# 192459/lmc-atomi

Hardware: AMD Instinct MI355X
Metric: lmc_chain_iterations_per_s (higher is better)
Workload: dtype f32; 1 GPU; 512x512 MYULA deblur (5x5 uniform box blur, sigma=0.75) + isotropic TV prox K=10 (tau_reg=0.3), 1024 chains/GPU x 1 GPU, Philox noise, x0=0, posterior moments every 1 it; chains_per_gpu=1024, chains_total=1024, tv_iters=10, sampler=MYULA (algs.py:477-587), parallelism=chains sharded x1, collective=none

## Files before the change

### lmc_atomi_amd/csrc/lmc_host.h

```cpp
#pragma once
#include <string>
#include <vector>

#include "lmc_launch.h"

namespace lmc::host {

int fail(int code, const char* fmt, ...);

#define HIP_TRY(expr)                                                                          \
  do {                                                                                         \
    hipError_t e_ = (expr);                                                                    \
    if (e_ != hipSuccess) return fail(LMC_E_HIP, "%s failed: %s", #expr, hipGetErrorString(e_)); \
  } while (0)

inline hipStream_t S(void* s) { return reinterpret_cast<hipStream_t>(s); }

inline bool eprox_params_ok(int kind, float p0, float p1) {
  static const unsigned char nonneg[] = {1, 1, 1, 1, 1, 1, 1, 3, 1, 1, 3, 1, 1, 0, 0};
  return (!(nonneg[kind] & 1) || p0 >= 0.f) && (!(nonneg[kind] & 2) || p1 >= 0.f);
}

struct Problem {
  int H = 0, W = 0;
  int data_kind = 0;
  int wl2 = 0;
  int pois = 0;
  float sigma_f = 0.f;
  const float* y = nullptr;
  const float* mask = nullptr;
  lmc::BlurTaps taps{};
  int prior_kind = 0;
  float prior_sigma = 0.f;
  int tv_niter = 0;
  float tv_step = 0.125f;
  float betas[lmc::kMaxTvIters] = {};
  int ncvx_kind = 0;
  float ncvx_lambda = 0.f, ncvx_gamma = 1.f;
  int ncvx_niter = 0;
  int ncvx_aniso = 0;
  int tv_warm = 0;
  int tv_warm_asked = 0;
  int tv_niter_asked = 0;
  float tv_rtol = 0.f;
  float ncvx_rtol = 0.f;
  int tv_exit_path = 0;
  int iters_per_launch = 0, moments_overlap = 0, moments_bg_wgs = 0;
  int cheb_pair = 1;
  int eprox_kind = 0, eprox_mask = 0;
  float eprox_p0 = 0.f, eprox_p1 = 0.f;
  const float* prox_scale = nullptr;
  int64_t prox_scale_cs = 0, prox_scale_ps = 0;
  int box = 0;
  float box_lo = 0.f, box_hi = 0.f;
  int variant = 0;
  float implicit_tol = 0.f;
};

struct RtState {
  int* kc = nullptr;
  int* start = nullptr;
  int* pred = nullptr;
  double* obj = nullptr;
  unsigned long long* reruns = nullptr;
  int stride = 0;
  size_t n = 0;
  hipError_t need(size_t n_img, int niter) {
    if (n_img <= n && niter + 1 <= stride) return hipSuccess;
    release();
    hipError_t e = hipMalloc(&kc, sizeof(int) * n_img);
    if (e == hipSuccess) e = hipMalloc(&start, sizeof(int) * n_img);
    if (e == hipSuccess) e = hipMalloc(&pred, sizeof(int) * n_img);
    if (e == hipSuccess) e = hipMalloc(&obj, sizeof(double) * n_img * (size_t)(niter + 1));
    if (e == hipSuccess) e = hipMalloc(&reruns, sizeof(unsigned long long) * 4);
    if (e == hipSuccess) e = hipMemset(pred, 0, sizeof(int) * n_img);
    if (e == hipSuccess) e = hipMemset(reruns, 0, sizeof(unsigned long long) * 4);
    if (e == hipSuccess) { n = n_img; stride = niter + 1; }
    return e;
  }
  void release() {
    if (kc) (void)hipFree(kc);
    if (start) (void)hipFree(start);
    if (pred) (void)hipFree(pred);
    if (obj) (void)hipFree(obj);
    if (reruns) (void)hipFree(reruns);
    kc = start = pred = nullptr; obj = nullptr; reruns = nullptr; n = 0; stride = 0;
  }
};

// ... 164 lines not shown
```

### lmc_atomi_amd/csrc/lmc_step_pipe.hip

```cpp
#include "lmc_step_pipe_kernel.h"

namespace lmc {

int centred_blur_taps(const StepArgs& a, float* uc, float* vc);

bool pipe_geometry_ok(const StepArgs& a) {
  if (a.prior_kind != LMC_PRIOR_TV_ISO || a.prox_ext) return false;
  if (a.W <= 128 || a.H < 1 || a.W > 16384) return false;
  if (a.W > 512 && (a.f_out || a.g_out)) return false;
  if ((a.W & (a.W > 256 ? 7 : 3)) && !(a.tv.niter == 10 || (a.tv.niter >= 20 && a.tv.niter % 10 == 0))) return false;
  if (a.data_kind == LMC_DATA_BLUR) {
    float uc[kMaxBlur], vc[kMaxBlur];
    if (centred_blur_taps(a, uc, vc) == 0) return false;
  } else if (a.data_kind != LMC_DATA_NONE && a.data_kind != LMC_DATA_IDENTITY && a.data_kind != LMC_DATA_MASK) {
    return false;
  }
  if (a.data_kind != LMC_DATA_BLUR && (a.ncvx_kind != LMC_NCVX_NONE || a.f_out)) return false;
  return true;
}

int pipe_links(const StepArgs& a) {
  if (a.prior_kind != LMC_PRIOR_TV_ISO || a.tv.niter > kMaxTvIters) return 0;
  const int n = a.tv.niter;
  const bool single = n == 2 || n == 6 || n == 8 || n == 9 || n == 10;
  if (!single && (n < 19 || (n % 10 != 0 && n % 10 != 9))) return 0;
  if (a.tv_aniso && (n % 10 != 0 || a.f_out || a.g_out)) return 0;
  if (a.box && (n % 10 != 0 || a.f_out || a.g_out || a.tv_aniso)) return 0;
  if (a.pois && (n != 10 || a.f_out || a.g_out || a.tv_aniso || a.ncvx_kind != LMC_NCVX_NONE || a.extra)) return 0;
  if (a.wl2 && (n != 10 || a.f_out || a.g_out || a.tv_aniso || a.ncvx_kind != LMC_NCVX_NONE || a.extra || a.data_kind == LMC_DATA_MASK)) return 0;
  if (a.tv_in || a.tv_out || a.tv_state_only || a.tv_warm) return 0;
  if (!pipe_geometry_ok(a)) return 0;
  return single ? 1 : (n + 9) / 10;
}

bool pipe_supported(const StepArgs& a) { return pipe_links(a) == 1; }

bool pipe_warm_supported(const StepArgs& a) {
  const int n = a.tv.niter;
  if (!(n == 1 || n == 2 || n == 3) || a.tv_aniso || a.box || a.pois || a.wl2) return false;
  return pipe_geometry_ok(a);
}

int pipe_taps(StepArgs& a) {
  int KT = 0;
  if (a.data_kind == LMC_DATA_BLUR) {
    float uc[kMaxBlur] = {0}, vc[kMaxBlur] = {0};
    KT = centred_blur_taps(a, uc, vc);
    for (int i = 0; i < kMaxBlur; ++i) { a.blur.h[i] = i < KT ? uc[i] : 0.f; a.blur.h[kMaxBlur + i] = i < KT ? vc[i] : 0.f; }
  }
  return KT;
}

hipError_t launch_step_pipe_warm(StepArgs a, hipStream_t st) {
  if (!pipe_warm_supported(a) || !a.tv_in || !a.tv_out || a.tv_in == a.tv_out) return hipErrorInvalidConfiguration;
  a.tv_warm = 1;
  a.tv_state_only = 0;
  const int KT = pipe_taps(a);
  return pipe_dispatch_chain(a, a.tv.niter, KT, st);
}

bool pipe_teams_covered(const StepArgs& a, int KT) {
  return a.tv.niter == 10 && KT == 5 && a.W >= 264 && a.W <= 512 && (a.W & 7) == 0 && !a.f_out && !a.g_out &&
         a.ncvx_kind == LMC_NCVX_NONE && !a.extra && !a.pois && !a.wl2;
}

hipError_t launch_step_pipe(StepArgs a, hipStream_t st, float* state0, float* state1, int teams) {
  const int links = pipe_links(a);
  if (links == 0 || (links > 1 && (!state0 || !state1))) return hipErrorInvalidConfiguration;
  const int KT = pipe_taps(a);
  const bool two = links == 1 && pipe_teams_covered(a, KT);
  if (teams == 2 && !two) return hipErrorInvalidConfiguration;
  if (a.pois) return links == 1 ? pipe_dispatch_pois(a, KT, st) : hipErrorInvalidConfiguration;
  if (a.wl2) return links == 1 ? pipe_dispatch_wl2(a, KT, st) : hipErrorInvalidConfiguration;
  if (a.tv_aniso) {
    if (two && teams != 1) return pipe_dispatch_aniso(a, KT, false, 2, st);
    if (links == 1) return pipe_dispatch_aniso(a, KT, false, 1, st);
  }
  if (a.box) {
    if (two && teams != 1) return pipe_dispatch_box(a, KT, false, 2, st);
    if (links == 1) return pipe_dispatch_box(a, KT, false, 1, st);
  }
  if (two && teams != 1) return pipe_launch_teams<10, 5>(a, st);
  if (links == 1) {
    switch (a.tv.niter) {
      case 2: return pipe_dispatch_k<2, false>(a, KT, st);
      case 6: return pipe_dispatch_k<6, false>(a, KT, st);
      case 8: return pipe_dispatch_k<8, false>(a, KT, st);
      case 9: return pipe_dispatch_k<9, false>(a, KT, st);
      default: return pipe_dispatch_k<10, false>(a, KT, st);
    }
  }
  float* st_buf[2] = {state0, state1};
  for (int j = 0; j < links; ++j) {
    StepArgs b = a;
    const int kl = (j == links - 1) ? a.tv.niter - 10 * j : 10;
    b.tv.niter = kl;
    for (int i = 0; i < kl; ++i) b.tv.betas[i] = a.tv.betas[10 * j + i];
    b.tv_in = j > 0 ? st_buf[(j - 1) & 1] : nullptr;
    b.tv_out = j < links - 1 ? st_buf[j & 1] : nullptr;
    b.tv_state_only = j < links - 1;
    const int ktl = b.tv_state_only ? 0 : KT;
    hipError_t e = a.tv_aniso ? pipe_dispatch_aniso(b, ktl, true, 1, st) : a.box ? pipe_dispatch_box(b, ktl, true, 1, st) : pipe_dispatch_chain(b, kl, ktl, st);
    if (e != hipSuccess) return e;
  }
  return hipSuccess;
}

}
```

### lmc_atomi_amd/csrc/lmc_step_pipe_kernel.h

```cpp
#pragma once
#include "lmc_device.h"
#include "lmc_launch.h"

namespace lmc {


template <int K>
struct PipeGeom {
  static constexpr int D = (2 * K + 2 > 10) ? 2 * K + 2 : 10;
  static constexpr int E = D - (2 * K + 2);
  static constexpr int RB = D + 1;
  static constexpr int NT = (K + 1) / 2;
};

template <int K, int PXL, bool CHAIN = false, int TEAMS = 1>
struct PipeLds {
  static constexpr int BW = 64 * PXL;
  static constexpr int RP = TEAMS * BW;
  static constexpr int o_x = 0;
  static constexpr int o_hand = o_x + PipeGeom<K>::RB * RP;
  static constexpr int o_hand_last = o_hand + (PipeGeom<K>::NT - 1) * 8 * RP;
  static constexpr int o_hand0 = o_hand_last + 4 * RP;
  static constexpr int o_g = CHAIN ? o_hand0 + 8 * RP : o_hand + PipeGeom<K>::NT * 2 * 4 * RP;
  static constexpr int SLAB = 2 * 4 * PXL * 64;
  static constexpr int o_slab = o_g + 2 * RP;
  static constexpr int o_seam = o_slab + TEAMS * SLAB;
  static constexpr int total = o_seam + (TEAMS == 2 ? 64 : 0);
};

template <int PXL>
__host__ __device__ constexpr int pipe_slot(int k) { return k < PXL / 2 ? 2 * k : 2 * (k - PXL / 2) + 1; }
template <int PXL>
__host__ __device__ constexpr int pipe_pixel(int s) { return (s >> 1) + (PXL / 2) * (s & 1); }
template <int PXL>
__host__ __device__ constexpr int pipe_slot_offset(int k) { return (pipe_slot<PXL>(k) >> 2) * 256 + (pipe_slot<PXL>(k) & 3); }
template <int PXL>
__device__ __forceinline__ void prow_load(float (&v)[PXL], const float* row, int lane) {
#pragma unroll
  for (int g = 0; g < PXL / 4; ++g) {
    const float4 q = *reinterpret_cast<const float4*>(row + g * 256 + lane * 4);
    v[pipe_pixel<PXL>(4 * g)] = q.x; v[pipe_pixel<PXL>(4 * g + 1)] = q.y; v[pipe_pixel<PXL>(4 * g + 2)] = q.z; v[pipe_pixel<PXL>(4 * g + 3)] = q.w;
  }
}
template <int PXL>
__device__ __forceinline__ void prow_store(float* row, int lane, const float (&v)[PXL]) {
#pragma unroll
  for (int g = 0; g < PXL / 4; ++g)
    *reinterpret_cast<float4*>(row + g * 256 + lane * 4) =
        make_float4(v[pipe_pixel<PXL>(4 * g)], v[pipe_pixel<PXL>(4 * g + 1)], v[pipe_pixel<PXL>(4 * g + 2)], v[pipe_pixel<PXL>(4 * g + 3)]);
}

typedef float v2f __attribute__((ext_vector_type(2)));
__device__ __forceinline__ v2f pk_fma(v2f a, v2f b, v2f c) { return __builtin_elementwise_fma(a, b, c); }
__device__ __forceinline__ v2f pk_set(float a) { return v2f{a, a}; }
__device__ __forceinline__ v2f pipe_clamp1(v2f a) { return v2f{__builtin_amdgcn_fmed3f(a.x, -1.f, 1.f), __builtin_amdgcn_fmed3f(a.y, -1.f, 1.f)}; }
__device__ __forceinline__ v2f pois_rho2(v2f u, v2f y, v2f beta) {
  const v2f den = v2f{fmaxf(u.x, 0.f), fmaxf(u.y, 0.f)} + beta, un = v2f{fminf(u.x, 0.f), fminf(u.y, 0.f)};
  const v2f t0 = v2f{__builtin_amdgcn_rcpf(den.x), __builtin_amdgcn_rcpf(den.y)};
  const v2f t = pk_fma(t0, pk_fma(-den, t0, pk_set(1.f)), t0);
  return pk_fma(-(y * t), pk_fma(-t, un, pk_set(1.f)), pk_set(1.f));
}
__device__ __forceinline__ v2f pipe_clamp_box(v2f a, float lo, float hi) { return v2f{__builtin_amdgcn_fmed3f(a.x, lo, hi), __builtin_amdgcn_fmed3f(a.y, lo, hi)}; }

template <int NP>
__device__ __forceinline__ void pairs_load(v2f (&v)[NP], const float* row, int lane) {
#pragma unroll
  for (int g = 0; g < NP / 2; ++g) {
    const float4 q = *reinterpret_cast<const float4*>(row + g * 256 + lane * 4);
    v[2 * g] = v2f{q.x, q.y};
    v[2 * g + 1] = v2f{q.z, q.w};
  }
}
template <int NP>
__device__ __forceinline__ void pairs_store(float* row, int lane, const v2f (&v)[NP]) {
#pragma unroll
  for (int g = 0; g < NP / 2; ++g)
    *reinterpret_cast<float4*>(row + g * 256 + lane * 4) = make_float4(v[2 * g].x, v[2 * g].y, v[2 * g + 1].x, v[2 * g + 1].y);
}

template <int NP>
__device__ __forceinline__ float pair_px(const v2f (&v)[NP], int k) { return k < NP ? v[k].x : v[k - NP].y; }
template <int NP>
__device__ __forceinline__ v2f left_pair(const v2f (&v)[NP], float from_left, int i) {
  if (i == 0) return v2f{from_left, v[NP - 1].x};
  return v[i - 1];
}
template <int NP>
__device__ __forceinline__ v2f right_pair(const v2f (&v)[NP], float from_right, int i) {
  if (i == NP - 1) return v2f{v[0].y, from_right};
  return v[i + 1];
}

template <int NP>
struct DualRow { v2f rr[NP], ss[NP], p[NP], q[NP]; };

__device__ __forceinline__ float wave_from_left(float v, float edge) {
  return __builtin_bit_cast(float, __builtin_amdgcn_update_dpp(__builtin_bit_cast(int, edge), __builtin_bit_cast(int, v), 0x138, 0xf, 0xf, false));
}
__device__ __forceinline__ float wave_from_right(float v, float edge) {
  return __builtin_bit_cast(float, __builtin_amdgcn_update_dpp(__builtin_bit_cast(int, edge), __builtin_bit_cast(int, v), 0x130, 0xf, 0xf, false));
}

template <int NP>
struct PipeCr { float cstep, cr_last; v2f ncrv[NP]; };
template <int NP, bool LASTLANE>
__device__ __forceinline__ v2f pipe_ncr(const PipeCr<NP>& c, int i) {
  if constexpr (LASTLANE) return i == NP - 1 ? v2f{-c.cstep, -c.cr_last} : pk_set(-c.cstep);
  else return c.ncrv[i];
}

struct StageObj { v2f sq, tv; };
template <int NP, bool PERPIX = false>
struct ObjMask {
  float md; v2f mlast;
  v2f mx[PERPIX ? NP : 1], my[PERPIX ? NP : 1];
};
template <int NP, bool LASTLANE>
__device__ __forceinline__ v2f obj_sq(const ObjMask<NP, !LASTLANE>* om, int i, v2f T) {
  if constexpr (LASTLANE) return T;
  else return T * om->mx[i];
}
template <int NP, bool LASTLANE>
__device__ __forceinline__ v2f obj_tv(const ObjMask<NP, !LASTLANE>* om, int i, v2f dxv, v2f dyv) {
  v2f dxm, dym;
  if constexpr (LASTLANE) { dxm = dxv * pk_set(om->md); dym = i == NP - 1 ? dyv * om->mlast : dyv; }
  else { dxm = dxv * pk_set(om->md) * om->mx[i]; dym = dyv * om->my[i]; }
  const v2f n = pk_fma(dxm, dxm, dym * dym);
  return v2f{__builtin_amdgcn_sqrtf(n.x), __builtin_amdgcn_sqrtf(n.y)};
}

template <int NP, bool LASTLANE = true, bool OBJ = false, bool SEAML = false, bool SEAMR = false, bool ANISO = false, bool BOX = false>
__device__ __forceinline__ void pipe_stage(const v2f (&xa)[NP], const v2f (&r1)[NP], const v2f (&s1)[NP], const DualRow<NP>& in0,
                                           v2f (&solb)[NP], float gam, float cdown, const PipeCr<NP>& cr, float beta,
                                           DualRow<NP>& out, StageObj* ob = nullptr, const ObjMask<NP, !LASTLANE>* om = nullptr,
                                           float ssl_edge = 0.f, float solr_edge = 0.f, float blo = 0.f, float bhi = 0.f) {
  v2f sol[NP];
  const float ssl0 = SEAML ? wave_from_left(s1[NP - 1].y, ssl_edge) : dpp_left0(s1[NP - 1].y);
  const v2f ngam = pk_set(-gam), ncd = pk_set(-cdown), vb = pk_set(beta);
#pragma unroll
  for (int i = 0; i < NP; ++i) {
    const v2f ssl = left_pair(s1, ssl0, i);
    const v2f T = (r1[i] - in0.rr[i]) + (s1[i] - ssl);
    sol[i] = pk_fma(ngam, T, xa[i]);
    if constexpr (BOX) sol[i] = pipe_clamp_box(sol[i], blo, bhi);
    if constexpr (OBJ) { const v2f Tm = obj_sq<NP, LASTLANE>(om, i, T); ob->sq = i == 0 ? Tm * Tm : pk_fma(Tm, Tm, ob->sq); }
  }
  const float solr_last = SEAMR ? wave_from_right(solb[0].x, solr_edge) : dpp_right0(solb[0].x);
#pragma unroll
  for (int i = 0; i < NP; ++i) {
    const v2f solr = right_pair(solb, solr_last, i);
    const v2f ncr = pipe_ncr<NP, LASTLANE>(cr, i);
    const v2f dxv = sol[i] - solb[i], dyv = solr - solb[i];
    if constexpr (OBJ) {
      const v2f nr = obj_tv<NP, LASTLANE>(om, i, dxv, dyv);
      ob->tv = i == 0 ? nr : ob->tv + nr;
    }
    const v2f r = pk_fma(ncd, dxv, in0.rr[i]);
    const v2f s = pk_fma(ncr, dyv, in0.ss[i]);
    v2f pn, qn;
    if constexpr (ANISO) {
      pn = pipe_clamp1(r);
      qn = pipe_clamp1(s);
    } else {
      const v2f n2 = pk_fma(r, r, s * s);
      const v2f inv = v2f{__builtin_amdgcn_fmed3f(__builtin_amdgcn_rsqf(n2.x), 0.f, 1.f), __builtin_amdgcn_fmed3f(__builtin_amdgcn_rsqf(n2.y), 0.f, 1.f)};
      pn = r * inv; qn = s * inv;
    }
    out.rr[i] = pk_fma(vb, pn - in0.p[i], pn);
    out.ss[i] = pk_fma(vb, qn - in0.q[i], qn);
    out.p[i] = pn;
    out.q[i] = qn;
  }
#pragma unroll
  for (int i = 0; i < NP; ++i) solb[i] = sol[i];
}

template <int NP, bool LASTLANE = true, bool OBJ = false, bool SEAMR = false, bool ANISO = false, bool BOX = false>
__device__ __forceinline__ void pipe_stage_first(const v2f (&xa)[NP], v2f (&solb)[NP], float cdown, const PipeCr<NP>& cr, float beta,
// ... 25 lines not shown
      qn = pipe_clamp1(s);
    } else {
      const v2f n2 = pk_fma(r, r, s * s);
      const v2f inv = v2f{__builtin_amdgcn_fmed3f(__builtin_amdgcn_rsqf(n2.x), 0.f, 1.f), __builtin_amdgcn_fmed3f(__builtin_amdgcn_rsqf(n2.y), 0.f, 1.f)};
      pn = r * inv; qn = s * inv;
    }
    out.rr[i] = pk_fma(vb, pn, pn);
    out.ss[i] = pk_fma(vb, qn, qn);
    out.p[i] = pn;
    out.q[i] = qn;
  }
#pragma unroll
  for (int i = 0; i < NP; ++i) solb[i] = x0(i);
}

template <int PXL>
__device__ __forceinline__ void gload_row(float (&dst)[PXL], const float* __restrict__ row, int c0, int W, bool ok, bool al = true) {
  if (al) {
#pragma unroll
    for (int g = 0; g < PXL / 4; ++g) {
      const bool okg = ok && c0 + 4 * g < W;
      const float4 v = *reinterpret_cast<const float4*>(row + (okg ? c0 + 4 * g : 0));
      dst[4 * g] = okg ? v.x : 0.f; dst[4 * g + 1] = okg ? v.y : 0.f; dst[4 * g + 2] = okg ? v.z : 0.f; dst[4 * g + 3] = okg ? v.w : 0.f;
    }
  } else {
#pragma unroll
    for (int g = 0; g < PXL / 4; ++g) {
      float v[4];
      load4_dword_aligned(v[0], v[1], v[2], v[3], row, c0 + 4 * g, W);
#pragma unroll
      for (int q = 0; q < 4; ++q) dst[4 * g + q] = (ok && c0 + 4 * g + q < W) ? v[q] : 0.f;
    }
  }
}

template <int PXL>
__device__ __forceinline__ void gload_raw(float (&dst)[PXL], const float* __restrict__ row, int c0, int W, bool al = true) {
  if (al) {
#pragma unroll
    for (int g = 0; g < PXL / 4; ++g) {
      const float4 v = *reinterpret_cast<const float4*>(row + (c0 + 4 * g < W ? c0 + 4 * g : 0));
      dst[4 * g] = v.x; dst[4 * g + 1] = v.y; dst[4 * g + 2] = v.z; dst[4 * g + 3] = v.w;
    }
  } else {
#pragma unroll
    for (int g = 0; g < PXL / 4; ++g) load4_dword_aligned_raw(dst[4 * g], dst[4 * g + 1], dst[4 * g + 2], dst[4 * g + 3], row, c0 + 4 * g, W);
  }
}
template <int PXL, bool AL>
__device__ __forceinline__ void gfix_raw(float (&r)[PXL], int c0, int W) {
  if constexpr (!AL) unshift_row_dword_aligned<PXL>(r, c0, W);
}

__device__ __forceinline__ void gstore4(float* __restrict__ row, int c, int lo, int hi, bool al, float v0, float v1, float v2, float v3) {
  if (al) {
    if (c >= lo && c < hi) *reinterpret_cast<float4*>(row + c) = make_float4(v0, v1, v2, v3);
  } else store4_dword_aligned(row, c, lo, hi, v0, v1, v2, v3);
}

__host__ __device__ constexpr int pipe_halo(int K, int KT, int PXL) {
  const int need = (K + 1 > KT - 1 ? K + 1 : KT - 1);
  return (need + PXL - 1) / PXL * PXL;
}

constexpr unsigned long long kPipe2Roles = 0xFCEDAB9687543210ull;
template <int K, int KT, bool CHAIN, bool RT>
__device__ __forceinline__ int pipe_role(int hw_wave, int kc, int ncvx_kind) {
  constexpr int NT = PipeGeom<K>::NT;
  if constexpr (K != 10) {
    return hw_wave;
  } else if constexpr (!RT) {
    const unsigned code = CHAIN ? 0x67325410u : ncvx_kind == LMC_NCVX_MC_TV ? 0x76354210u : (KT == 7 ? 0x75264310u : 0x76325410u);
    return (code >> (4 * hw_wave)) & 15;
  } else {
    if (kc <= NT) {
      const unsigned code = kc >= 5 ? 0x76543210u : kc == 4 ? 0x67514320u : 0x64753210u;
      return (code >> (4 * hw_wave)) & 15;
    }
    if (CHAIN) return (0x67254310u >> (4 * hw_wave)) & 15;
    return hw_wave == 4 ? 6 : hw_wave == 6 ? 4 : hw_wave;
  }
}

template <int K, int PXL, int KT, bool CHAIN, bool WARM, bool AL, bool RT, int TEAMS, bool ANISO = false, bool BOX = false, bool POIS = false, bool WL2 = false>
__device__ __forceinline__ void pipe_body(const StepArgs& A) {
  static_assert(!WL2 || (TEAMS == 1 && !CHAIN && !WARM && !RT && !ANISO && K == 10 && !POIS),
                "weighted Gaussian data term: one team, one launch of 10 dual iterations, isotropic prior, not with the Poisson term");
  static_assert(!POIS || (TEAMS == 1 && !CHAIN && !WARM && !RT && !ANISO && K == 10), "Poisson data term: one team, one launch of 10 dual iterations, isotropic prior");
  static_assert(!WARM || CHAIN, "the warm dual uses the state hand-over of the chained launches");
  static_assert(!ANISO || (!WARM && !RT), "anisotropic prior: the early exit's objective and the warm dual are not built");
  static_assert(!BOX || (!WARM && !RT), "box constraint: the early exit's objective and the warm dual are not built");
  constexpr bool kStateInN = (ANISO || BOX) && CHAIN && KT > 0 && PXL == 8;
  static_assert(!RT || (!WARM && (K & 1) == 0), "per-chain exit: cold start, even K");
  static_assert(!RT || AL || pipe_halo(K, KT, PXL) >= K + 2, "per-chain exit on column strips: the halo holds the objective's extra column");
  static_assert(TEAMS == 1 || (TEAMS == 2 && K == 10 && PXL == 4 && KT == 5 && AL && !CHAIN && !WARM && !RT),
                "two teams: one fixed-count launch, 5 taps, aligned rows, 4 pixels per lane");
  using G = PipeGeom<K>;
  using L = PipeLds<K, PXL, CHAIN, TEAMS>;
  constexpr int D = G::D, E = G::E, RB = G::RB, NT = G::NT, BW = L::BW, RP = L::RP, HW = KT > 0 ? (KT - 1) / 2 : 0;
  constexpr int LAGT = TEAMS == 2 ? 1 : 0;
  static_assert(K >= 1, "at least one dual iteration");
  static_assert(D >= KT + 1 + LAGT, "the blur pipeline reads ring rows at least one tick old");
  extern __shared__ float lds_all[];
  const int lane = threadIdx.x & 63;
  const int hw_wave = __builtin_amdgcn_readfirstlane(threadIdx.x >> 6);
  const int chain = blockIdx.x;
  const int H = A.H, W = A.W;
  int kc = K;
  bool state_only = CHAIN && A.tv_state_only;
  if constexpr (RT) {
    const int kc_g = __builtin_amdgcn_readfirstlane(A.rt_kc[chain]);
    if (kc_g <= A.rt_base) return;
    if (CHAIN && A.rt_start && A.rt_base < K * (__builtin_amdgcn_readfirstlane(A.rt_start[chain]) & 0xFFFF)) return;
    kc = min(kc_g - A.rt_base, K);
    state_only = CHAIN && kc_g > A.rt_base + K;
  }
  int team = 0, wave;
  if constexpr (TEAMS == 2) {
    const unsigned nib = (unsigned)(kPipe2Roles >> (4 * hw_wave)) & 15u;
    team = nib >> 3;
    wave = nib & 7;
  } else {
    wave = pipe_role<K, KT, CHAIN, RT>(hw_wave, kc, A.ncvx_kind);
  }
  constexpr int HALO = pipe_halo(K, KT, PXL);
  const int strip = blockIdx.y;
  const int strip_u = gridDim.y > 1 ? BW - 2 * HALO : W;
  int c0 = (strip ? strip * strip_u - HALO : 0) + lane * PXL;
  int st_lo = strip * strip_u, st_hi = min(W, st_lo + strip_u);
  if constexpr (TEAMS == 2) {
    const int Wt = W >> 1;
    c0 = team ? Wt + lane * PXL : Wt - BW + lane * PXL;
    st_lo = team ? Wt : 0;
    st_hi = team ? W : Wt;
  }
  const bool cok = c0 >= st_lo && c0 < st_hi;
  const int cl = TEAMS == 2 ? (cok ? c0 : 0) : c0;
  auto col_in = [&](int k) __attribute__((always_inline)) -> bool { return TEAMS == 2 ? cok : c0 + k < W; };
  constexpr bool al = AL;
  const size_t img = (size_t)H * W;
  const float* __restrict__ xin = A.x_in + (size_t)chain * img;
  float* __restrict__ xout = A.x_out + (size_t)chain * img;

  for (int e = threadIdx.x; e < L::total; e += blockDim.x) lds_all[e] = 0.f;
  __syncthreads();
  float* const lds = lds_all + team * BW;
  float* const slab_base = lds_all + L::o_slab + team * L::SLAB;
  float* const seam = lds_all + L::o_seam;
  constexpr int SA = 0, SB = 4 * (NT + 1), SR = SB + 4 * NT;
  static_assert(TEAMS == 1 || SR + 8 <= L::total - L::o_seam, "seam records");

  const int T_end = (H + D + 3) & ~3;
  float* const xring = lds + L::o_x;
  auto ring_row = [&](int row) -> float* { return xring + ((unsigned)(row + RB) % (unsigned)RB) * RP; };

  constexpr int kPrioL = 3, kPrioC = 3, kPrioT = 1, kPrioN = 0;
  if (wave == 0) __builtin_amdgcn_s_setprio(kPrioL);
  else if (wave == NT + 1) __builtin_amdgcn_s_setprio(kPrioC);
  else if (wave <= NT) __builtin_amdgcn_s_setprio(kPrioT);
  else __builtin_amdgcn_s_setprio(kPrioN);
  auto roles = [&](auto team_tag) __attribute__((always_inline)) {
  constexpr int TM = decltype(team_tag)::value;
  if (wave == 0) {
    const float* __restrict__ uv = A.blur.h;
    constexpr bool kRing4 = (KT == 5);
    constexpr int NWIN = KT > 1 ? KT - 1 : 1;
    constexpr int kXPF = 4;
    constexpr int NP = PXL / 2;
    float xpre[kXPF][PXL], ypre[4][PXL];
    float bpre[POIS || WL2 ? 4 : 1][POIS || WL2 ? PXL : 1];
    v2f hxw[NWIN][NP], hrw[NWIN][NP];
    constexpr int kYPF = (KT == 7 || TEAMS == 2) ? 2 : 3;
#pragma unroll
    for (int a = 0; a < NWIN; ++a)
#pragma unroll
      for (int k = 0; k < NP; ++k) { hxw[a][k] = pk_set(0.f); hrw[a][k] = pk_set(0.f); }
#pragma unroll
    for (int u = 0; u < kXPF; ++u) gload_raw<PXL>(xpre[u], xin + (size_t)min(u, H - 1) * W, cl, W, al);
    if constexpr (KT > 0) {
#pragma unroll
      for (int u = 0; u < kYPF; ++u) {
        const int r = u + 1 - D + (KT - 1) - HW + LAGT;
        gload_raw<PXL>(ypre[u], A.y + (size_t)min(max(r, 0), H - 1) * W, cl, W, al);
        if constexpr (POIS || WL2) gload_raw<PXL>(bpre[u], A.y + img + (size_t)min(max(r, 0), H - 1) * W, cl, W, al);
      }
    }
    const bool pw_id = KT == 0 && A.data_kind == LMC_DATA_IDENTITY, pw_mask = KT == 0 && A.data_kind == LMC_DATA_MASK;
    float mpre[KT == 0 ? 4 : 1][KT == 0 ? PXL : 1];
    if constexpr (KT == 0) {
#pragma unroll
      for (int u = 0; u < 4; ++u)
#pragma unroll
        for (int k = 0; k < PXL; ++k) { ypre[u][k] = 0.f; mpre[u][k] = 0.f; }
      if constexpr (POIS || WL2) {
#pragma unroll
        for (int u = 0; u < 4; ++u)
#pragma unroll
          for (int k = 0; k < PXL; ++k) bpre[u][k] = 1.f;
      }
      if (pw_id || pw_mask) {
#pragma unroll
        for (int u = 0; u < kYPF; ++u) {
          const size_t ro = (size_t)min(max(u + 1 - D, 0), H - 1) * W;
          gload_raw<PXL>(ypre[u], A.y + ro, c0, W, al);
          if constexpr (POIS || WL2) gload_raw<PXL>(bpre[u], A.y + img + ro, c0, W, al);
          if (pw_mask) gload_raw<PXL>(mpre[u], A.mask + ro, c0, W, al);
        }
      }
    }
    constexpr int nsf = CHAIN ? (WARM ? 2 : 4) : 0;
    constexpr int kSPF = 2;
    float spre[CHAIN ? kSPF : 1][CHAIN ? nsf : 1][CHAIN ? PXL : 1];
    const float* const sin = CHAIN && A.tv_in ? A.tv_in + (size_t)chain * nsf * img : nullptr;
    if constexpr (CHAIN && !kStateInN) {
#pragma unroll
      for (int u = 0; u < kSPF; ++u) {
        const int rs = u - E - 1;
#pragma unroll
        for (int f = 0; f < nsf; ++f)
          gload_raw<PXL>(spre[u][f], sin ? sin + (size_t)f * img + (size_t)min(max(rs, 0), H - 1) * W : xin, c0, W, al);
      }
    }
    double facc = 0.0;
    v2f Rprev[TEAMS == 2 ? NP : 1];
#pragma unroll
    for (int k = 0; k < (TEAMS == 2 ? NP : 1); ++k) Rprev[k] = pk_set(0.f);
    auto tick = [&](auto uu, const int t) __attribute__((always_inline)) {
      constexpr int U = decltype(uu)::value, P = U & 1;
      if constexpr (KT > 0) {
        const int r3 = t + kYPF + 1 - D + (KT - 1) - HW + LAGT;
        gload_raw<PXL>(ypre[(U + kYPF) & 3], A.y + (size_t)min(max(r3, 0), H - 1) * W, cl, W, al);
        if constexpr (POIS || WL2) gload_raw<PXL>(bpre[(U + kYPF) & 3], A.y + img + (size_t)min(max(r3, 0), H - 1) * W, cl, W, al);
      } else if (pw_id || pw_mask) {
        const size_t ro = (size_t)min(max(t + kYPF + 1 - D, 0), H - 1) * W;
        gload_raw<PXL>(ypre[(U + kYPF) & 3], A.y + ro, c0, W, al);
        if constexpr (POIS || WL2) gload_raw<PXL>(bpre[(U + kYPF) & 3], A.y + img + ro, c0, W, al);
        if (pw_mask) gload_raw<PXL>(mpre[(U + kYPF) & 3], A.mask + ro, c0, W, al);
      }
      {
        float xv[PXL];
        gfix_raw<PXL, AL>(xpre[U], c0, W);
#pragma unroll
        for (int k = 0; k < PXL; ++k) xv[k] = (t < H && col_in(k)) ? xpre[U][k] : 0.f;
        prow_store<PXL>(ring_row(t), lane, xv);
        gload_raw<PXL>(xpre[U], xin + (size_t)min(t + kXPF, H - 1) * W, cl, W, al);
      }
      if constexpr (CHAIN && !kStateInN) {
        float* hb = lds + L::o_hand0 + P * 4 * RP;
        constexpr int SP = U & (kSPF - 1);
        const int rh = t - E - 1;
        const bool rowok_h = sin && rh >= 0 && rh < H;
#pragma unroll
        for (int f = 0; f < nsf; ++f) {
          gfix_raw<PXL, AL>(spre[SP][f], c0, W);
          float sv[PXL];
#pragma unroll
          for (int k = 0; k < PXL; ++k) sv[k] = (rowok_h && c0 + (AL ? (k & ~3) : k) < W) ? spre[SP][f][k] : 0.f;
          prow_store<PXL>(hb + f * RP, lane, sv);
        }
        const int rs = t + kSPF - E - 1;
#pragma unroll
        for (int f = 0; f < nsf; ++f)
          gload_raw<PXL>(spre[SP][f], sin ? sin + (size_t)f * img + (size_t)min(max(rs, 0), H - 1) * W : xin, c0, W, al);
      }
      if constexpr (KT > 0) {
      const int i = t + 1 - D + (KT - 1) + LAGT;
      v2f hxn[NP];
      {
        v2f xi[NP];
        float e[PXL + 2 * HW];
        const float* const xr = ring_row(i);
        pairs_load<NP>(xi, xr, lane);
#pragma unroll
        for (int m = 0; m < HW; ++m)
          e[m] = (TEAMS == 2 && TM == 1) ? wave_from_left(pair_px<NP>(xi, PXL - HW + m), xr[63 * 4 + pipe_slot_offset<PXL>(PXL - HW + m) - BW])
                                         : dpp_left0(pair_px<NP>(xi, PXL - HW + m));
#pragma unroll
        for (int k = 0; k < PXL; ++k) e[HW + k] = pair_px<NP>(xi, k);
#pragma unroll
        for (int m = 0; m < HW; ++m)
          e[HW + PXL + m] = (TEAMS == 2 && TM == 0) ? wave_from_right(pair_px<NP>(xi, m), xr[BW + pipe_slot_offset<PXL>(m)]) : dpp_right0(pair_px<NP>(xi, m));
#pragma unroll
        for (int j = 0; j < NP; ++j) {
          v2f acc = pk_set(uv[kMaxBlur]) * v2f{e[j + 2 * HW], e[j + 2 * HW + NP]};
#pragma unroll
          for (int b = 1; b < KT; ++b) acc = pk_fma(pk_set(uv[kMaxBlur + b]), v2f{e[j + 2 * HW - b], e[j + 2 * HW - b + NP]}, acc);
          hxn[j] = acc;
        }
      }
      const int r = i - HW;
      v2f R[NP];
      {
        const bool rowok = r >= 0 && r < H;
        const float rmask = rowok ? 1.f : 0.f;
        gfix_raw<PXL, AL>(ypre[U & 3], c0, W);
        if constexpr (POIS || WL2) gfix_raw<PXL, AL>(bpre[U & 3], c0, W);
#pragma unroll
        for (int j = 0; j < NP; ++j) {
          v2f acc = pk_set(uv[0]) * hxn[j];
#pragma unroll
          for (int a = 1; a < KT; ++a) acc = pk_fma(pk_set(uv[a]), hxw[kRing4 ? ((U - a) & 3) : a - 1][j], acc);
          v2f d;
          if constexpr (POIS) d = pois_rho2(acc, v2f{ypre[U & 3][j], ypre[U & 3][j + NP]}, v2f{bpre[U & 3][j], bpre[U & 3][j + NP]});
          else d = v2f{acc.x - ypre[U & 3][j], acc.y - ypre[U & 3][j + NP]};
          if constexpr (WL2) d = d * v2f{bpre[U & 3][j], bpre[U & 3][j + NP]};
          R[j] = d * v2f{(TEAMS == 2 ? cok : AL ? c0 < W : c0 + j < W) ? rmask : 0.f, (TEAMS == 2 ? cok : AL ? c0 < W : c0 + j + NP < W) ? rmask : 0.f};
        }
        if (TEAMS == 1 && A.f_out) {
#pragma unroll
          for (int k = 0; k < PXL; ++k) facc = fma((double)pair_px<NP>(R, k), (double)pair_px<NP>(R, k), facc);
        }
        if constexpr (!kRing4) {
#pragma unroll
          for (int a = KT - 2; a >= 1; --a)
#pragma unroll
            for (int j = 0; j < NP; ++j) hxw[a][j] = hxw[a - 1][j];
        }
#pragma unroll
        for (int j = 0; j < NP; ++j) hxw[kRing4 ? (U & 3) : 0][j] = hxn[j];
      }
      if constexpr (TEAMS == 2) {
        if (TM == 0 ? lane == 63 : lane == 0) {
#pragma unroll
          for (int m = 0; m < HW; ++m) seam[SR + P * 4 + 2 * TM + m] = pair_px<NP>(R, TM == 0 ? PXL - HW + m : m);
        }
#pragma unroll
        for (int j = 0; j < NP; ++j) { const v2f tmp = R[j]; R[j] = Rprev[j]; Rprev[j] = tmp; }
      }
      {
        float e[PXL + 2 * HW];
        v2f gout[NP];
        const float* const sr = seam + SR + (P ^ 1) * 4;
#pragma unroll
        for (int m = 0; m < HW; ++m)
          e[m] = (TEAMS == 2 && TM == 1) ? wave_from_left(pair_px<NP>(R, PXL - HW + m), sr[m]) : dpp_left0(pair_px<NP>(R, PXL - HW + m));
#pragma unroll
        for (int k = 0; k < PXL; ++k) e[HW + k] = pair_px<NP>(R, k);
#pragma unroll
        for (int m = 0; m < HW; ++m) e[HW + PXL + m] = (TEAMS == 2 && TM == 0) ? wave_from_right(pair_px<NP>(R, m), sr[2 + m]) : dpp_right0(pair_px<NP>(R, m));
#pragma unroll
        for (int j = 0; j < NP; ++j) {
          v2f hrn = pk_set(uv[kMaxBlur]) * v2f{e[j], e[j + NP]};
#pragma unroll
          for (int b = 1; b < KT; ++b) hrn = pk_fma(pk_set(uv[kMaxBlur + b]), v2f{e[j + b], e[j + b + NP]}, hrn);
          v2f acc = pk_set(uv[KT - 1]) * hrn;
#pragma unroll
          for (int a = 0; a < KT - 1; ++a) acc = pk_fma(pk_set(uv[a]), hrw[kRing4 ? ((U - (KT - 1 - a)) & 3) : KT - 2 - a][j], acc);
          if constexpr (!kRing4) {
#pragma unroll
            for (int a = KT - 2; a >= 1; --a) hrw[a][j] = hrw[a - 1][j];
          }
          hrw[kRing4 ? (U & 3) : 0][j] = hrn;
          gout[j] = pk_set(A.sigma_f) * acc;
        }
        pairs_store<NP>(lds + L::o_g + P * RP, lane, gout);
      }
      }
      if constexpr (KT == 0) {
        if (pw_id || pw_mask) {
          const int i = t + 1 - D;
          float xi[PXL], gout[PXL];
          prow_load<PXL>(xi, ring_row(i), lane);
          const bool rowok = i >= 0 && i < H;
          gfix_raw<PXL, AL>(ypre[U & 3], c0, W);
          if (pw_mask) gfix_raw<PXL, AL>(mpre[U & 3], c0, W);
          if constexpr (POIS || WL2) gfix_raw<PXL, AL>(bpre[U & 3], c0, W);
#pragma unroll
          for (int k = 0; k < PXL; ++k) {
            float g = 0.f;
            if (rowok && c0 + k < W) {
              if constexpr (POIS) {
                if (pw_id) g = A.sigma_f * pois_rho(xi[k], ypre[U & 3][k], bpre[U & 3][k]);
                else g = A.sigma_f * mpre[U & 3][k] * pois_rho(mpre[U & 3][k] * xi[k], ypre[U & 3][k], bpre[U & 3][k]);
              } else if constexpr (WL2) {
                g = A.sigma_f * (bpre[U & 3][k] * (xi[k] - ypre[U & 3][k]));
              } else {
              if (pw_id) g = A.sigma_f * (xi[k] - ypre[U & 3][k]);
              else g = A.sigma_f * mpre[U & 3][k] * fmaf(mpre[U & 3][k], xi[k], -ypre[U & 3][k]);
              }
            }
            gout[k] = g;
          }
          prow_store<PXL>(lds + L::o_g + P * RP, lane, gout);
        }
      }
      __syncthreads();
    };
    for (int t = 0; t < T_end; t += 4) static_for<0, 4>([&](auto uu) { tick(uu, t + decltype(uu)::value); });
    if (TEAMS == 1 && A.f_out) {
      const double tot = wave_sum(facc);
      if (lane == 0) unsafeAtomicAdd(&A.f_out[chain], 0.5 * (double)A.sigma_f * tot);
    }
  } else if (wave <= NT) {
    auto t_role = [&](auto first_tag, auto single_tag) __attribute__((always_inline)) {
    constexpr bool FIRST = decltype(first_tag)::value;
    constexpr bool SINGLE = decltype(single_tag)::value;
    const int k1 = 2 * wave - 1, k2 = 2 * wave;
    const bool spread = RT && kc <= NT;
    const int g1 = spread ? wave : k1, g2 = k2;
    const float gam = A.tv.gamma, cstep = A.tv.c;
    const float blo = BOX ? A.box_lo : 0.f, bhi = BOX ? A.box_hi : 0.f;
    const float beta1 = A.tv.betas[g1 - 1], beta2 = SINGLE ? 0.f : A.tv.betas[g2 - 1];
    PipeCr<PXL / 2> crc;
    crc.cstep = cstep;
    crc.cr_last = (c0 + PXL - 1 == W - 1 || (TEAMS == 2 && !cok)) ? 0.f : cstep;
#pragma unroll
    for (int i = 0; i < PXL / 2; ++i) crc.ncrv[i] = v2f{c0 + i == W - 1 ? 0.f : -cstep, c0 + i + PXL / 2 == W - 1 ? 0.f : -cstep};
    float* const hout = lds + L::o_hand + (wave - 1) * 8 * RP;
    const bool from_state = CHAIN && wave == 1 && A.tv_in != nullptr;
    constexpr bool warm = WARM;
    const float* const hin = from_state ? lds + L::o_hand0 : hout - 8 * RP;
    constexpr int nof = warm ? 2 : 4;
    float* const sout = CHAIN && wave == NT && A.tv_out && (!RT || state_only) ? A.tv_out + (size_t)chain * nof * img : nullptr;
    constexpr int NP = PXL / 2;
    const bool live1 = !RT || g1 <= kc, live2 = !RT || (!spread && g2 <= kc);
    const bool fullpass2 = spread && wave < kc;
    ObjMask<NP, !AL> om;
    om.md = 0.f;
    om.mlast = v2f{1.f, (c0 + PXL - 1 == W - 1) ? 0.f : 1.f};
    if constexpr (RT && !AL) {
#pragma unroll
      for (int i = 0; i < NP; ++i) {
        const int ca = c0 + i, cb = ca + NP;
        const bool ina = ca >= st_lo && ca < st_hi, inb_ = cb >= st_lo && cb < st_hi;
        om.mx[i] = v2f{ina ? 1.f : 0.f, inb_ ? 1.f : 0.f};
        om.my[i] = v2f{ina && ca < W - 1 ? 1.f : 0.f, inb_ && cb < W - 1 ? 1.f : 0.f};
      }
    }
    double osq1 = 0.0, otv1 = 0.0, osq2 = 0.0, otv2 = 0.0;
    DualRow<NP> inb[2], o1[2];
    v2f sol1[NP], sol2[NP];
    v2f xk[2][NP];
#pragma unroll
    for (int k = 0; k < NP; ++k) {
      sol1[k] = sol2[k] = pk_set(0.f);
      xk[0][k] = xk[1][k] = pk_set(0.f);
// ... 410 lines not shown
}

template <int K, int PXL, int KT, bool CHAIN = false, bool WARM = false, bool AL = true, bool RT = false>
__global__ __launch_bounds__(64 * ((K + 1) / 2 + 3), (PXL == 8 || CHAIN) ? 1 : 2) void myula_step_pipe_kernel(const StepArgs A) {
  pipe_body<K, PXL, KT, CHAIN, WARM, AL, RT, 1>(A);
}

template <int K, int KT>
__global__ __launch_bounds__(128 * ((K + 1) / 2 + 3), 4) void myula_step_pipe2_kernel(const StepArgs A) {
  pipe_body<K, 4, KT, false, false, true, false, 2>(A);
}


template <int K, int PXL, int KT, bool CHAIN = false>
static constexpr size_t pipe_lds_bytes() { return sizeof(float) * (size_t)PipeLds<K, PXL, CHAIN>::total; }
template <int K>
static constexpr size_t pipe_teams_lds_bytes() { return sizeof(float) * (size_t)PipeLds<K, 4, false, 2>::total; }
static_assert(pipe_teams_lds_bytes<10>() <= 160 * 1024, "LDS of one workgroup");

template <auto Kern>
static hipError_t pipe_launch(size_t lds_bytes, dim3 grid, dim3 block, const StepArgs& a, hipStream_t st) {
  static bool attr_set[64] = {};
  int dev = 0;
  hipError_t e = hipGetDevice(&dev);
  if (e != hipSuccess) return e;
  if (dev < 0 || dev >= 64 || !attr_set[dev]) {
    e = hipFuncSetAttribute(reinterpret_cast<const void*>(Kern), hipFuncAttributeMaxDynamicSharedMemorySize, (int)lds_bytes);
    if (e != hipSuccess) return e;
    if (dev >= 0 && dev < 64) attr_set[dev] = true;
  }
  hipLaunchKernelGGL(Kern, grid, block, lds_bytes, st, a);
  return hipGetLastError();
}

template <int K, int PXL, int KT>
static int pipe_nstrips(int W) {
  constexpr int BWk = 64 * PXL, U = BWk - 2 * pipe_halo(K, KT, PXL);
  return W <= BWk ? 1 : (W + U - 1) / U;
}
constexpr int pipe_block(int K, int teams) { return 64 * teams * ((K + 1) / 2 + 3); }

static bool pipe_lastlane(int W) { return (W & (W > 256 ? 7 : 3)) == 0; }

template <class F>
static hipError_t pipe_select(int W, int KT, F&& f) {
  auto taps = [&](auto pxl) {
    if (KT == 5) return f(pxl, std::integral_constant<int, 5>{});
    if (KT == 7) return f(pxl, std::integral_constant<int, 7>{});
    return f(pxl, std::integral_constant<int, 0>{});
  };
  return W > 256 ? taps(std::integral_constant<int, 8>{}) : taps(std::integral_constant<int, 4>{});
}

template <int PXL, int KT, bool CHAIN, int K = 10, bool WARM = false, bool AL = true, bool RT = false>
static hipError_t pipe_launch_one(const StepArgs& a, hipStream_t st) {
  return pipe_launch<myula_step_pipe_kernel<K, PXL, KT, CHAIN, WARM, AL, RT>>(pipe_lds_bytes<K, PXL, KT, CHAIN>(), dim3(a.C, pipe_nstrips<K, PXL, KT>(a.W)),
                                                                              dim3(pipe_block(K, 1)), a, st);
}

template <int K, int KT>
static hipError_t pipe_launch_teams(const StepArgs& a, hipStream_t st) {
  return pipe_launch<myula_step_pipe2_kernel<K, KT>>(pipe_teams_lds_bytes<K>(), dim3(a.C), dim3(pipe_block(K, 2)), a, st);
}

template <int K, bool CHAIN, bool WARM = false>
static hipError_t pipe_dispatch_k(const StepArgs& a, int KT, hipStream_t st) {
  return pipe_select(a.W, KT, [&](auto pxl, auto kt) {
    constexpr int PXL = decltype(pxl)::value, KTc = decltype(kt)::value;
    if (pipe_lastlane(a.W)) return pipe_launch_one<PXL, KTc, CHAIN, K, WARM>(a, st);
    if constexpr (K == 10 && !WARM) return pipe_launch_one<PXL, KTc, CHAIN, K, false, false>(a, st);
    else return hipErrorInvalidConfiguration;
  });
}

bool pipe_geometry_ok(const StepArgs& a);
int pipe_taps(StepArgs& a);

hipError_t pipe_dispatch_chain(const StepArgs& a, int K, int KT, hipStream_t st);

hipError_t pipe_dispatch_box(const StepArgs& a, int KT, bool chain, int teams, hipStream_t st);

hipError_t pipe_dispatch_aniso(const StepArgs& a, int KT, bool chain, int teams, hipStream_t st);

hipError_t pipe_dispatch_pois(const StepArgs& a, int KT, hipStream_t st);

hipError_t pipe_dispatch_wl2(const StepArgs& a, int KT, hipStream_t st);

}
```

### lmc_atomi_amd/csrc/lmc_step_rows.hip

```cpp
#include "lmc_step_rows_kernel.h"

#include <cmath>
#include <cstdlib>

namespace lmc {

hipError_t launch_step_rows_uni(const StepArgs& a, int KT, int lo, int hi, bool al, int nblk, int band, int nbands, hipStream_t st, bool* handled);

bool separate_blur_taps(const BlurTaps& T, float* u, float* v) {
  int pa = 0, pb = 0;
  float best = 0.f;
  for (int a = 0; a < T.kh; ++a)
    for (int b = 0; b < T.kw; ++b)
      if (fabsf(T.h[a * T.kw + b]) > best) { best = fabsf(T.h[a * T.kw + b]); pa = a; pb = b; }
  if (best == 0.f) return false;
  const float piv = T.h[pa * T.kw + pb];
  for (int a = 0; a < T.kh; ++a) u[a] = T.h[a * T.kw + pb] / piv;
  for (int b = 0; b < T.kw; ++b) v[b] = T.h[pa * T.kw + b];
  for (int a = 0; a < T.kh; ++a)
    for (int b = 0; b < T.kw; ++b)
      if (fabsf(u[a] * v[b] - T.h[a * T.kw + b]) > 1e-6f * best) return false;
  return true;
}

static bool rows_centre(const float* u, int n, int off, int KT, float* out) {
  const int HW = (KT - 1) / 2, sh = HW - off;
  if (sh < 0 || n + sh > KT) return false;
  for (int i = 0; i < KT; ++i) out[i] = 0.f;
  for (int i = 0; i < n; ++i) out[i + sh] = u[i];
  return true;
}

int centred_blur_taps(const BlurTaps& T, float* uc, float* vc) {
  float u[kMaxBlur] = {0}, v[kMaxBlur] = {0};
  if (T.kh > 7 || T.kw > 7 || !separate_blur_taps(T, u, v)) return 0;
  for (int KT = 5; KT <= 7; KT += 2)
    if (rows_centre(u, T.kh, T.oy, KT, uc) && rows_centre(v, T.kw, T.ox, KT, vc)) return KT;
  return 0;
}
int centred_blur_taps(const StepArgs& a, float* uc, float* vc) { return centred_blur_taps(a.blur, uc, vc); }

bool rows_supported(const StepArgs& a) {
  if (a.data_kind != LMC_DATA_BLUR || a.ncvx_kind != LMC_NCVX_NONE) return false;
  if (a.prior_kind != LMC_PRIOR_NONE && a.prior_kind != LMC_PRIOR_L2 && a.prior_kind != LMC_PRIOR_L1 && a.prior_kind != LMC_PRIOR_EPROX) return false;
  if (a.prior_kind == LMC_PRIOR_EPROX && ((a.W & 3) || a.W > 512 || a.dot_out)) return false;
  if (a.tv_in || a.tv_out) return false;
  if (a.W < 4 || a.W > 16384 || a.H < 1) return false;
  float uc[kMaxBlur], vc[kMaxBlur];
  const int KT = centred_blur_taps(a, uc, vc);
  if (KT == 0) return false;
  return true;
}

hipError_t launch_step_rows(StepArgs a, hipStream_t st) {
  if (!rows_supported(a)) return hipErrorInvalidConfiguration;
  float uc[kMaxBlur] = {0}, vc[kMaxBlur] = {0};
  const int KT = centred_blur_taps(a, uc, vc);
  for (int i = 0; i < kMaxBlur; ++i) { a.blur.h[i] = i < KT ? uc[i] : 0.f; a.blur.h[kMaxBlur + i] = i < KT ? vc[i] : 0.f; }
  static const int env_band = [] { const char* e = getenv("LMC_ROWS_BAND"); return e ? atoi(e) : 0; }();
  int band = env_band > 0 ? env_band : 0;
  if (band == 0) {
    const int want = (4096 + a.C - 1) / a.C;
    band = (a.H + want - 1) / want;
    if (band < 16) band = 16;
  }
  band = (band + 7) & ~7;
  const int nbands = (a.H + band - 1) / band;
  const bool al = (a.W & 3) == 0;
  const int pxl = (a.W <= 256 && al) ? 4 : 8;
  const int ustrip = 64 * pxl - 16;
  const int nstrips = a.W <= 64 * pxl ? 1 : (a.W + ustrip - 1) / ustrip;
  const long long waves = (long long)a.C * nbands * nstrips;
  if (waves > (1ll << 31) - 8) return hipErrorInvalidConfiguration;
  const int nblk = (int)((waves + 3) / 4);
  if (a.dot_out) {
    if (!al) {
      if (KT == 5) hipLaunchKernelGGL((myula_step_rows_kernel<8, 5, true, -1, -1, false>), dim3(nblk), dim3(256), 0, st, a, band, nbands);
      else hipLaunchKernelGGL((myula_step_rows_kernel<8, 7, true, -1, -1, false>), dim3(nblk), dim3(256), 0, st, a, band, nbands);
    } else if (a.W <= 256) {
      if (KT == 5) hipLaunchKernelGGL((myula_step_rows_kernel<4, 5, true>), dim3(nblk), dim3(256), 0, st, a, band, nbands);
      else hipLaunchKernelGGL((myula_step_rows_kernel<4, 7, true>), dim3(nblk), dim3(256), 0, st, a, band, nbands);
    } else {
      if (KT == 5) hipLaunchKernelGGL((myula_step_rows_kernel<8, 5, true>), dim3(nblk), dim3(256), 0, st, a, band, nbands);
      else hipLaunchKernelGGL((myula_step_rows_kernel<8, 7, true>), dim3(nblk), dim3(256), 0, st, a, band, nbands);
    }
    return hipGetLastError();
  }
  auto window = [&](const float* t, int& l, int& h) {
    l = -1; h = -1;
    for (int i = 0; i < KT; ++i) if (t[i] != 0.f) { if (l < 0) l = i; h = i; }
    if (l < 0) return false;
    for (int i = l; i <= h; ++i) if (std::fabs(t[i] - t[l]) > 1e-6f * std::fabs(t[l])) return false;
    return true;
  };
  int lo = -1, hi = -1, l2, h2;
  if (!(window(uc, lo, hi) && window(vc, l2, h2) && l2 == lo && h2 == hi)) lo = hi = -1;
  {
    bool handled = false;
    const hipError_t e = launch_step_rows_uni(a, KT, lo, hi, al, nblk, band, nbands, st, &handled);
    if (handled) return e;
  }
  if (!al) {
    if (KT == 5) hipLaunchKernelGGL((myula_step_rows_kernel<8, 5, false, -1, -1, false>), dim3(nblk), dim3(256), 0, st, a, band, nbands);
    else hipLaunchKernelGGL((myula_step_rows_kernel<8, 7, false, -1, -1, false>), dim3(nblk), dim3(256), 0, st, a, band, nbands);
  } else if (a.W <= 256) {
    if (KT == 5) hipLaunchKernelGGL((myula_step_rows_kernel<4, 5>), dim3(nblk), dim3(256), 0, st, a, band, nbands);
    else hipLaunchKernelGGL((myula_step_rows_kernel<4, 7>), dim3(nblk), dim3(256), 0, st, a, band, nbands);
  } else {
    if (KT == 5) hipLaunchKernelGGL((myula_step_rows_kernel<8, 5>), dim3(nblk), dim3(256), 0, st, a, band, nbands);
    else hipLaunchKernelGGL((myula_step_rows_kernel<8, 7>), dim3(nblk), dim3(256), 0, st, a, band, nbands);
  }
  return hipGetLastError();
}

}
```

Before: 611,700 chain-it/s.

## Add uniform-box specialization of pipelined MYULA step using running sums

```diff
diff --git a/lmc_atomi_amd/csrc/lmc_host.h b/lmc_atomi_amd/csrc/lmc_host.h
--- a/lmc_atomi_amd/csrc/lmc_host.h
+++ b/lmc_atomi_amd/csrc/lmc_host.h
@@ -1,10 +1,19 @@
 #pragma once
+#include <cmath>
 #include <string>
 #include <vector>
 
 #include "lmc_launch.h"
 
 namespace lmc::host {
+
+inline bool uniform_window(const float* t, int KT, int& lo, int& hi) {
+  lo = -1; hi = -1;
+  for (int i = 0; i < KT; ++i) if (t[i] != 0.f) { if (lo < 0) lo = i; hi = i; }
+  if (lo < 0) return false;
+  for (int i = lo; i <= hi; ++i) if (std::fabs(t[i] - t[lo]) > 1e-6f * std::fabs(t[lo])) return false;
+  return true;
+}
 
 int fail(int code, const char* fmt, ...);
 
diff --git a/lmc_atomi_amd/csrc/lmc_step_pipe.hip b/lmc_atomi_amd/csrc/lmc_step_pipe.hip
--- a/lmc_atomi_amd/csrc/lmc_step_pipe.hip
+++ b/lmc_atomi_amd/csrc/lmc_step_pipe.hip
@@ -1,3 +1,4 @@
+#include "lmc_host.h"
 #include "lmc_step_pipe_kernel.h"
 
 namespace lmc {
@@ -64,6 +65,13 @@
          a.ncvx_kind == LMC_NCVX_NONE && !a.extra && !a.pois && !a.wl2;
 }
 
+bool pipe_uni_covered(const StepArgs& a, int KT) {
+  if (!(a.tv.niter == 10 && KT == 5 && a.W <= 512 && pipe_lastlane(a.W))) return false;
+  if (a.tv_aniso || a.box || a.pois || a.wl2 || a.f_out || a.g_out || a.ncvx_kind != LMC_NCVX_NONE || a.extra || a.rt_kc || a.tv_warm) return false;
+  int lo, hi, l2, h2;
+  return host::uniform_window(a.blur.h, KT, lo, hi) && host::uniform_window(a.blur.h + kMaxBlur, KT, l2, h2) && lo == 0 && hi == 4 && l2 == 0 && h2 == 4;
+}
+
 hipError_t launch_step_pipe(StepArgs a, hipStream_t st, float* state0, float* state1, int teams) {
   const int links = pipe_links(a);
   if (links == 0 || (links > 1 && (!state0 || !state1))) return hipErrorInvalidConfiguration;
@@ -80,6 +88,7 @@
     if (two && teams != 1) return pipe_dispatch_box(a, KT, false, 2, st);
     if (links == 1) return pipe_dispatch_box(a, KT, false, 1, st);
   }
+  if (links == 1 && pipe_uni_covered(a, KT)) return pipe_dispatch_uni(a, KT, two && teams != 1 ? 2 : 1, st);
   if (two && teams != 1) return pipe_launch_teams<10, 5>(a, st);
   if (links == 1) {
     switch (a.tv.niter) {
diff --git a/lmc_atomi_amd/csrc/lmc_step_pipe_kernel.h b/lmc_atomi_amd/csrc/lmc_step_pipe_kernel.h
--- a/lmc_atomi_amd/csrc/lmc_step_pipe_kernel.h
+++ b/lmc_atomi_amd/csrc/lmc_step_pipe_kernel.h
@@ -94,6 +94,17 @@
 template <int NP>
 struct DualRow { v2f rr[NP], ss[NP], p[NP], q[NP]; };
 
+template <int NP>
+__device__ __forceinline__ void uni_hsum(const float (&e)[2 * NP + 4], v2f (&out)[NP]) {
+  v2f E[NP + 4], A[NP + 2];
+#pragma unroll
+  for (int m = 0; m < NP + 4; ++m) E[m] = v2f{e[m], e[m + NP]};
+#pragma unroll
+  for (int m = 0; m < NP + 2; ++m) A[m] = E[m] + E[m + 1];
+#pragma unroll
+  for (int j = 0; j < NP; ++j) out[j] = (A[j] + A[j + 2]) + E[j + 4];
+}
+
 __device__ __forceinline__ float wave_from_left(float v, float edge) {
   return __builtin_bit_cast(float, __builtin_amdgcn_update_dpp(__builtin_bit_cast(int, edge), __builtin_bit_cast(int, v), 0x138, 0xf, 0xf, false));
 }
@@ -285,8 +296,11 @@
   }
 }
 
-template <int K, int PXL, int KT, bool CHAIN, bool WARM, bool AL, bool RT, int TEAMS, bool ANISO = false, bool BOX = false, bool POIS = false, bool WL2 = false>
+template <int K, int PXL, int KT, bool CHAIN, bool WARM, bool AL, bool RT, int TEAMS, bool ANISO = false, bool BOX = false, bool POIS = false, bool WL2 = false,
+          bool UNI = false>
 __device__ __forceinline__ void pipe_body(const StepArgs& A) {
+  static_assert(!UNI || (K == 10 && KT == 5 && AL && !CHAIN && !WARM && !RT && !ANISO && !BOX && !POIS && !WL2),
+                "uniform-box form: one fixed-count launch of 10 dual iterations, 5 taps, aligned rows, plain Gaussian data term, isotropic prior");
   static_assert(!WL2 || (TEAMS == 1 && !CHAIN && !WARM && !RT && !ANISO && K == 10 && !POIS),
                 "weighted Gaussian data term: one team, one launch of 10 dual iterations, isotropic prior, not with the Poisson term");
   static_assert(!POIS || (TEAMS == 1 && !CHAIN && !WARM && !RT && !ANISO && K == 10), "Poisson data term: one team, one launch of 10 dual iterations, isotropic prior");
@@ -373,6 +387,12 @@
     float xpre[kXPF][PXL], ypre[4][PXL];
     float bpre[POIS || WL2 ? 4 : 1][POIS || WL2 ? PXL : 1];
     v2f hxw[NWIN][NP], hrw[NWIN][NP];
+    v2f hxp[UNI ? 2 : 1][NP], hrp[UNI ? 2 : 1][NP];
+    const float cbox = UNI ? uv[0] * uv[kMaxBlur] : 0.f;
+#pragma unroll
+    for (int a = 0; a < (UNI ? 2 : 1); ++a)
+#pragma unroll
+      for (int k = 0; k < NP; ++k) { hxp[a][k] = pk_set(0.f); hrp[a][k] = pk_set(0.f); }
     constexpr int kYPF = (KT == 7 || TEAMS == 2) ? 2 : 3;
 #pragma unroll
     for (int a = 0; a < NWIN; ++a)
@@ -483,12 +503,16 @@
 #pragma unroll
         for (int m = 0; m < HW; ++m)
           e[HW + PXL + m] = (TEAMS == 2 && TM == 0) ? wave_from_right(pair_px<NP>(xi, m), xr[BW + pipe_slot_offset<PXL>(m)]) : dpp_right0(pair_px<NP>(xi, m));
+        if constexpr (UNI) {
+          uni_hsum<NP>(e, hxn);
+        } else {
 #pragma unroll
         for (int j = 0; j < NP; ++j) {
           v2f acc = pk_set(uv[kMaxBlur]) * v2f{e[j + 2 * HW], e[j + 2 * HW + NP]};
 #pragma unroll
           for (int b = 1; b < KT; ++b) acc = pk_fma(pk_set(uv[kMaxBlur + b]), v2f{e[j + 2 * HW - b], e[j + 2 * HW - b + NP]}, acc);
           hxn[j] = acc;
+        }
         }
       }
       const int r = i - HW;
@@ -500,11 +524,17 @@
         if constexpr (POIS || WL2) gfix_raw<PXL, AL>(bpre[U & 3], c0, W);
 #pragma unroll
         for (int j = 0; j < NP; ++j) {
-          v2f acc = pk_set(uv[0]) * hxn[j];
+          v2f acc;
+          if constexpr (UNI) {
+            acc = (hxn[j] + hxw[(U - 1) & 3][j]) + hxw[(U - 3) & 3][j];
+          } else {
+          acc = pk_set(uv[0]) * hxn[j];
 #pragma unroll
           for (int a = 1; a < KT; ++a) acc = pk_fma(pk_set(uv[a]), hxw[kRing4 ? ((U - a) & 3) : a - 1][j], acc);
+          }
           v2f d;
           if constexpr (POIS) d = pois_rho2(acc, v2f{ypre[U & 3][j], ypre[U & 3][j + NP]}, v2f{bpre[U & 3][j], bpre[U & 3][j + NP]});
+          else if constexpr (UNI) d = v2f{__builtin_fmaf(cbox, acc.x, -ypre[U & 3][j]), __builtin_fmaf(cbox, acc.y, -ypre[U & 3][j + NP])};
           else d = v2f{acc.x - ypre[U & 3][j], acc.y - ypre[U & 3][j + NP]};
           if constexpr (WL2) d = d * v2f{bpre[U & 3][j], bpre[U & 3][j + NP]};
           R[j] = d * v2f{(TEAMS == 2 ? cok : AL ? c0 < W : c0 + j < W) ? rmask : 0.f, (TEAMS == 2 ? cok : AL ? c0 < W : c0 + j + NP < W) ? rmask : 0.f};
@@ -520,7 +550,10 @@
             for (int j = 0; j < NP; ++j) hxw[a][j] = hxw[a - 1][j];
         }
 #pragma unroll
-        for (int j = 0; j < NP; ++j) hxw[kRing4 ? (U & 3) : 0][j] = hxn[j];
+        for (int j = 0; j < NP; ++j) {
+          if constexpr (UNI) { hxw[U & 3][j] = hxn[j] + hxp[P ^ 1][j]; hxp[P][j] = hxn[j]; }
+          else hxw[kRing4 ? (U & 3) : 0][j] = hxn[j];
+        }
       }
       if constexpr (TEAMS == 2) {
         if (TM == 0 ? lane == 63 : lane == 0) {
@@ -541,6 +574,17 @@
         for (int k = 0; k < PXL; ++k) e[HW + k] = pair_px<NP>(R, k);
 #pragma unroll
         for (int m = 0; m < HW; ++m) e[HW + PXL + m] = (TEAMS == 2 && TM == 0) ? wave_from_right(pair_px<NP>(R, m), sr[2 + m]) : dpp_right0(pair_px<NP>(R, m));
+        if constexpr (UNI) {
+          v2f hrn[NP];
+          uni_hsum<NP>(e, hrn);
+#pragma unroll
+          for (int j = 0; j < NP; ++j) {
+            const v2f acc = (hrn[j] + hrw[(U - 1) & 3][j]) + hrw[(U - 3) & 3][j];
+            hrw[U & 3][j] = hrn[j] + hrp[P ^ 1][j];
+            hrp[P][j] = hrn[j];
+            gout[j] = pk_set(A.sigma_f * cbox) * acc;
+          }
+        } else {
 #pragma unroll
         for (int j = 0; j < NP; ++j) {
           v2f hrn = pk_set(uv[kMaxBlur]) * v2f{e[j], e[j + NP]};
@@ -555,6 +599,7 @@
           }
           hrw[kRing4 ? (U & 3) : 0][j] = hrn;
           gout[j] = pk_set(A.sigma_f) * acc;
+        }
         }
         pairs_store<NP>(lds + L::o_g + P * RP, lane, gout);
       }
@@ -1131,6 +1176,8 @@
 
 hipError_t pipe_dispatch_aniso(const StepArgs& a, int KT, bool chain, int teams, hipStream_t st);
 
+hipError_t pipe_dispatch_uni(const StepArgs& a, int KT, int teams, hipStream_t st);
+
 hipError_t pipe_dispatch_pois(const StepArgs& a, int KT, hipStream_t st);
 
 hipError_t pipe_dispatch_wl2(const StepArgs& a, int KT, hipStream_t st);
diff --git a/lmc_atomi_amd/csrc/lmc_step_pipe_uni.hip b/lmc_atomi_amd/csrc/lmc_step_pipe_uni.hip
--- /dev/null
+++ b/lmc_atomi_amd/csrc/lmc_step_pipe_uni.hip
@@ -0,0 +1,27 @@
+#include "lmc_step_pipe_kernel.h"
+
+namespace lmc {
+
+template <int K, int PXL, int KT>
+__global__ __launch_bounds__(64 * ((K + 1) / 2 + 3), PXL == 8 ? 1 : 2) void myula_step_pipe_uni_kernel(const StepArgs A) {
+  pipe_body<K, PXL, KT, false, false, true, false, 1, false, false, false, false, true>(A);
+}
+
+template <int K, int KT>
+__global__ __launch_bounds__(128 * ((K + 1) / 2 + 3), 4) void myula_step_pipe_uni2_kernel(const StepArgs A) {
+  pipe_body<K, 4, KT, false, false, true, false, 2, false, false, false, false, true>(A);
+}
+
+template <int PXL>
+static hipError_t pipe_uni_launch_one(const StepArgs& a, hipStream_t st) {
+  constexpr int K = 10;
+  return pipe_launch<myula_step_pipe_uni_kernel<K, PXL, 5>>(pipe_lds_bytes<K, PXL, 5, false>(), dim3(a.C), dim3(pipe_block(K, 1)), a, st);
+}
+
+hipError_t pipe_dispatch_uni(const StepArgs& a, int KT, int teams, hipStream_t st) {
+  if (a.tv.niter != 10 || KT != 5 || !pipe_lastlane(a.W) || a.W > 512 || a.tv_warm || a.tv_aniso || a.box || a.pois || a.wl2 || a.rt_kc) return hipErrorInvalidConfiguration;
+  if (teams == 2) return pipe_launch<myula_step_pipe_uni2_kernel<10, 5>>(pipe_teams_lds_bytes<10>(), dim3(a.C), dim3(pipe_block(10, 2)), a, st);
+  return a.W > 256 ? pipe_uni_launch_one<8>(a, st) : pipe_uni_launch_one<4>(a, st);
+}
+
+}
diff --git a/lmc_atomi_amd/csrc/lmc_step_rows.hip b/lmc_atomi_amd/csrc/lmc_step_rows.hip
--- a/lmc_atomi_amd/csrc/lmc_step_rows.hip
+++ b/lmc_atomi_amd/csrc/lmc_step_rows.hip
@@ -1,3 +1,4 @@
+#include "lmc_host.h"
 #include "lmc_step_rows_kernel.h"
 
 #include <cmath>
@@ -86,15 +87,8 @@
     }
     return hipGetLastError();
   }
-  auto window = [&](const float* t, int& l, int& h) {
-    l = -1; h = -1;
-    for (int i = 0; i < KT; ++i) if (t[i] != 0.f) { if (l < 0) l = i; h = i; }
-    if (l < 0) return false;
-    for (int i = l; i <= h; ++i) if (std::fabs(t[i] - t[l]) > 1e-6f * std::fabs(t[l])) return false;
-    return true;
-  };
   int lo = -1, hi = -1, l2, h2;
-  if (!(window(uc, lo, hi) && window(vc, l2, h2) && l2 == lo && h2 == hi)) lo = hi = -1;
+  if (!(host::uniform_window(uc, KT, lo, hi) && host::uniform_window(vc, KT, l2, h2) && l2 == lo && h2 == hi)) lo = hi = -1;
   {
     bool handled = false;
     const hipError_t e = launch_step_rows_uni(a, KT, lo, hi, al, nblk, band, nbands, st, &handled);
```

Result: faster. 621,700 chain-it/s (median of 6 runs) (+1.6%).
